# fzaiser/genfer

Measured on AMD Instinct MI355X. Metric: TaylorPoly mul f64 GMAC/s, higher is better.
Workload: dtype f64

## Files before the change

### genfer_amd/csrc/gft_api.hip

```cpp
#include <hip/hip_runtime.h>
#include <dlfcn.h>
#include <rccl/rccl.h>

#include <algorithm>
#include <chrono>
#include <atomic>
#include <cmath>
#include <cstdio>
#include <cstring>
#include <deque>
#include <exception>
#include <functional>
#include <initializer_list>
#include <map>
#include <memory>
#include <tuple>
#include <stdexcept>
#include <string>
#include <vector>

#include "../../include/gftaylor.h"
#include "gft_kernels.hpp"
#include "gft_small_alloc.hpp"
#include "gft_host.hpp"
// ... 1257 lines not shown
        HIP_OK(hipEventSynchronize(R.events[b]));
        float ms = 0;
        HIP_OK(hipEventElapsedTime(&ms, R.events[a], R.events[b]));
        return ms;
    } catch (const std::exception& e) {
        g_err = e.what();
        return -1.0f;
    }
}
int gft_set_option(const char* name, double value) {
    std::string n = name ? name : "";
    if (n == "horner_loop_max") R.horner_loop_max = value < 0 ? 0 : (size_t)value;
    else if (n == "div_wavefront") R.div_wavefront = value != 0;
    else if (n == "exp_right") R.exp_right = value != 0;
    else if (n == "recur_overlap") R.recur_overlap = value != 0;
    else if (n == "defer") R.defer = value != 0;
    else if (n == "lazy_observe") R.lazy_observe = value != 0;
    else if (n == "batch_dag") R.batch_dag = value != 0;
    else if (n == "lazy_horner") R.lazy_horner = value != 0;
    else if (n == "nz_proofs") R.nz_proofs = value != 0;
    else if (n == "lazy_sum") R.lazy_sum = value != 0;
    else if (n == "async_launch") lq_configure(R.device, value != 0);
    else if (n == "trace_lq_report") lq_report();
    else if (n == "shallow_max_terms") R.shallow_max_terms = value < 0 ? 256 : (size_t)value;
    else if (n == "debug_fail_next_launch") g_fail_next_launch.store(value != 0 ? 1 : 0);
    else if (n == "tiled_min_macs") R.tiled_min_macs = value;
    else if (n == "conv_rb_min_macs") staged_set_rb_min_macs(value);
    else if (n == "conv_rb_pairs") staged_set_rb_pairs(value);
    else if (n == "conv_rb_pairs_cap") staged_set_rb_pairs_cap(value);
    else if (n == "conv_rb_pairs_lanes") staged_set_rb_pairs_lanes(value);
    else if (n == "shallow_pair_min") shallow_set_pair_min(value == -1.0 ? 4096.0 : value);
    else if (n == "tiled_tile") tiled_set_lane_tile((int)value);
    else if (n == "tiled_peel") tiled_set_peel((int)value);
    else if (n == "tiled_peel_lanes") tiled_set_peel_lanes((int)value);
    else if (n == "tiled_slots") tiled_set_slots((int)value);
    else if (n == "tiled_taper") tiled_set_taper((int)value);
    else if (n == "host_max_elems") R.host_max_elems = value < 0 ? Runtime::HOST_MAX_ELEMS_DEFAULT : (size_t)value;
    else if (n == "host_max_macs") R.host_max_macs = value < 0 ? Runtime::HOST_MAX_MACS_DEFAULT : value;
    else if (n == "series_form") R.series_force = (value == 1 || value == 2) ? (int)value : 0;
    else if (n == "dist_min_macs") dist_set_min_macs(value);
    else if (n == "dist_event_slot") dist_set_event_slot(value);
    else return -1;
    return 0;
}
int gft_set_conv_variant(int v) {
    R.conv_variant = v;
    return 0;
}
int gft_set_conv_mode(int mode) {
    if (mode < 0 || mode > 3) return -1;
    R.conv_mode = mode;
    return 0;
}

int gft_conv_raw(const double* x, const size_t* xshape, const double* y, const size_t* yshape, double* res,
                 const size_t* rshape, size_t ndim, size_t slab_lo, size_t slab_hi, int accumulate) {
    return guard_int([&] {
        typedef Ops<EF64> O;
        O::HV xv{const_cast<double*>(x), 0, dims(xshape, ndim)};
        O::HV yv{const_cast<double*>(y), 0, dims(yshape, ndim)};
        O::HV zv{res, 0, dims(rshape, ndim)};
        for (size_t i = 0; i < ndim; ++i)
            if (xshape[i] > rshape[i] || yshape[i] > rshape[i] || xshape[i] == 0 || yshape[i] == 0)
                throw Error("conv_raw: operand shapes must be non-empty and not exceed the result shape");
        if (ndim > 0 && (slab_lo > slab_hi || slab_hi > rshape[0])) throw Error("conv_raw: bad slab range");
        O::conv(xv, yv, zv, slab_lo, slab_hi, accumulate != 0, false, 0, 0, 0);
// ... 581 lines not shown
```

### genfer_amd/csrc/gft_conv_tiled.hip

```cpp
#include <algorithm>
#include <cstdio>
#include <cstdlib>
#include <cstring>
#include <map>
#include <vector>

#include "gft_kernels.hpp"
#include "gft_peel_layout.hpp"

namespace gft {

namespace {

struct TileSeg {
    unsigned u, a, b;
    unsigned step_begin, step_end;
    int dest;
};

struct RedTile {
    unsigned u, a, b;
    unsigned first, count;
    unsigned slot0;
};
// ... 13 lines not shown
    unsigned cut;
    unsigned lim1;
    size_t zsU, zs0, zs1, zoff;
    const double* xp;
    const double* yp;
    double* z;
    double* ws;
    const TileSeg* segs;
    const unsigned* wg_begin;
    const RedTile* red;
    const unsigned* red_slots;
    const unsigned* guard;
    unsigned guard_epoch;
    unsigned* claim;
    unsigned n_ranges, n_queues;
#ifdef GFT_TILED_DIAG
    unsigned long long* stamps;
#endif
    unsigned char blk1[8], blk2[8];
};

typedef const double __attribute__((address_space(4))) * cptr_t;

#ifndef GFT_TILED_DEFAULT_VARIANT
#define GFT_TILED_DEFAULT_VARIANT 7
#endif
#ifndef GFT_TILED_PEEL_DEFAULT
#define GFT_TILED_PEEL_DEFAULT -1
#endif
#ifndef GFT_TILED_PEEL_LANES_DEFAULT
#define GFT_TILED_PEEL_LANES_DEFAULT -1
#endif
constexpr unsigned PEEL_MIN_EXTENT = 112, PEEL_MIN_INNER = 64;

__device__ inline void loadx(double (&dst)[8], cptr_t p) {
#pragma unroll
    for (int i = 0; i < 8; ++i) dst[i] = p[i];
}

__device__ inline void load8(double (&dst)[8], const double* p) {
#pragma unroll
    for (int i = 0; i < 8; ++i) dst[i] = p[i];
}

__device__ inline void load8_b128(double (&dst)[8], const double* p) {
    const double2* q = reinterpret_cast<const double2*>(__builtin_assume_aligned(p, 16));
#pragma unroll
    for (int i = 0; i < 4; ++i) {
        double2 v = q[i];
        dst[2 * i] = v.x;
        dst[2 * i + 1] = v.y;
    }
}

__device__ inline void fma_rows(double (&acc)[8], const double (&xq)[8], const double (&cur)[8],
                                const double (&prev)[8], int s_lo, int s_hi) {
#pragma unroll
    for (int s = 0; s < 8; ++s) {
        if (s < s_lo || s >= s_hi) continue;
        const double xs = xq[s];
#pragma unroll
        for (int r = 0; r < 8; ++r) {
            const double yv = (r - s >= 0) ? cur[(r - s) & 7] : prev[(8 + r - s) & 7];
            acc[r] = __builtin_fma(xs, yv, acc[r]);
        }
    }
// ... 449 lines not shown
                                                   double* __restrict__ w0, double* __restrict__ s1, double* __restrict__ w1,
                                                   unsigned n0, unsigned n1, unsigned nI, unsigned n8) {
    const size_t t0 = (size_t)7 * (n0 / 8) * n1 * n8, ts = (size_t)7 * n0 * n8, t1 = (size_t)7 * (n1 / 8) * n0 * n8;
    for (size_t i = blockIdx.x * (size_t)blockDim.x + threadIdx.x; i < t0 + ts + t1; i += (size_t)gridDim.x * blockDim.x) {
        const double* src;
        double* dst;
        size_t row;
        unsigned col;
        if (i < t0) {
            row = i / n8;
            col = (unsigned)(i - row * n8);
            const unsigned r1 = (unsigned)(row % n1), va = (unsigned)(row / n1), a = va % (n0 / 8), v = va / (n0 / 8);
            src = x + ((size_t)(8 * a + 1 + v) * n1 + r1) * nI;
            dst = w0 + i;
        } else if (i < t0 + ts) {
            const size_t k = i - t0;
            row = k / n8;
            col = (unsigned)(k - row * n8);
            const unsigned j1c = (unsigned)(row % n0), ju = (unsigned)(row / n0);
            src = y + ((size_t)j1c * n1 + ju) * nI;
            dst = s1 + k;
        } else {
            const size_t k = i - t0 - ts;
            row = k / n8;
            col = (unsigned)(k - row * n8);
            const unsigned r = (unsigned)(row % n0), vb = (unsigned)(row / n0), b = vb % (n1 / 8), v = vb / (n1 / 8);
            src = x + ((size_t)r * n1 + 8 * b + 1 + v) * nI;
            dst = w1 + k;
        }
        *dst = col < nI ? src[col] : 0.0;
    }
}

__global__ void __launch_bounds__(256) k_pad_rows(const double* __restrict__ in, double* __restrict__ out, size_t rows,
                                                  unsigned len, unsigned P, unsigned B) {
    const size_t per_p = rows * B, total = per_p * P;
    for (size_t i = blockIdx.x * (size_t)blockDim.x + threadIdx.x; i < total; i += (size_t)gridDim.x * blockDim.x) {
        const unsigned p = (unsigned)(i / per_p);
        const size_t rem = i - (size_t)p * per_p, row = rem / B;
        const unsigned col = p * B + (unsigned)(rem - row * B);
        out[i] = col < len ? in[row * len + col] : 0.0;
    }
}
__global__ void __launch_bounds__(256) k_fold_rows(const double* __restrict__ zt, double* __restrict__ z, size_t rows,
                                                   size_t row_lo, size_t row_hi, unsigned Pz, unsigned B, unsigned zI,
                                                   int accumulate, const unsigned* guard, unsigned epoch) {
    if (guard && *guard == epoch) return;
    const unsigned RI = 2 * B - 1;
    size_t total = (row_hi - row_lo) * zI;
    for (size_t i = blockIdx.x * (size_t)blockDim.x + threadIdx.x; i < total; i += (size_t)gridDim.x * blockDim.x) {
        size_t row = row_lo + i / zI;
        unsigned k = (unsigned)(i % zI), p = k / B, r = k - p * B;
        double v = p < Pz ? zt[((size_t)p * rows + row) * RI + r] : 0.0;
        if (p > 0 && p - 1 < Pz && r + 1 < B) v += zt[((size_t)(p - 1) * rows + row) * RI + B + r];
        double* dst = z + row * zI + k;
        *dst = accumulate ? *dst + v : v;
    }
}


struct Variant {
    bool fast;
    bool b128;
    bool xcd;
    bool compact;
    bool peel;
// ... 62 lines not shown
}

unsigned long long& plan_generation() {
    static unsigned long long g = 0;
    return g;
}

void reset_plan_cache(hipStream_t st) {
    (void)hipStreamSynchronize(st);
    for (auto& kv : plan_cache())
        if (kv.second.d_tables) (void)hipFree(kv.second.d_tables);
    plan_cache().clear();
    plan_generation()++;
    arena().head = 0;
}

int num_cus() {
    static int n = 0;
    if (!n) {
        int dev = 0;
        (void)hipGetDevice(&dev);
        hipDeviceProp_t p;
        if (hipGetDeviceProperties(&p, dev) == hipSuccess) n = p.multiProcessorCount;
        if (n <= 0) n = 256;
    }
    return n;
}

struct PeelSpec {
    unsigned role = 0;
    unsigned cut = 0, lim1 = 0;
    size_t zsU = 0, zs0 = 0, zs1 = 0, zoff = 0;
    unsigned all_slabs = 0;
};

int& tiled_slots_cap() {
    static int v = 0;
    return v;
}
#ifndef GFT_TILED_TAPER_DEFAULT
#define GFT_TILED_TAPER_DEFAULT 80
#endif
int& tiled_taper_pct() {
    static int v = GFT_TILED_TAPER_DEFAULT;
    return v;
}

int& tiled_force_tsh() {
    static int v = 0;
    return v;
}

unsigned pick_lane_tile(const TiledArgs& T) {
    auto axis_eff = [](unsigned T, unsigned nx, unsigned ny, unsigned nz) {
        double useful = 0, issued = 0;
        for (unsigned t = 0; t * T < nz; ++t) {
            const unsigned kmax = std::min(T * t + T - 1, nz - 1);
            const unsigned jlo = T * t + 1 > ny ? T * t + 1 - ny : 0, jhi = std::min(kmax + 1, nx);
            if (jhi > jlo) issued += (double)(jhi - jlo) * T;
            for (unsigned k = T * t; k <= kmax; ++k) {
                const unsigned lo = k + 1 > ny ? k + 1 - ny : 0, hi = std::min(k + 1, nx);
                if (hi > lo) useful += hi - lo;
            }
        }
        return issued > 0 ? useful / issued : 0.0;
    };
// ... 275 lines not shown
        case 1: launch_main_nw<1, VAR>(st, P, T, grid); break;
        case 2: launch_main_nw<2, VAR>(st, P, T, grid); break;
        case 4: launch_main_nw<4, VAR>(st, P, T, grid); break;
        default: launch_main_nw<8, VAR>(st, P, T, grid); break;
    }
}

}

void tiled_pad_rows_f64(hipStream_t st, const double* in, double* out, size_t rows, unsigned len, unsigned P, unsigned B) {
    size_t tot = rows * P * B;
    if (!tot) return;
    GFT_LAUNCH(k_pad_rows, dim3((unsigned)std::min<size_t>((tot + 255) / 256, 4096)), dim3(256), 0, st, in, out, rows,
                       len, P, B);
}
void tiled_fold_rows_f64(hipStream_t st, const double* zt, double* z, size_t rows, size_t row_lo, size_t row_hi, unsigned Pz,
                         unsigned B, unsigned zI, int accumulate, const unsigned* guard, unsigned epoch) {
    size_t tot = (row_hi - row_lo) * zI;
    if (!tot) return;
    GFT_LAUNCH(k_fold_rows, dim3((unsigned)std::min<size_t>((tot + 255) / 256, 4096)), dim3(256), 0, st, zt, z, rows,
                       row_lo, row_hi, Pz, B, zI, accumulate, guard, epoch);
}

void tiled_set_lane_tile(int tsh) { tiled_force_tsh() = tsh; }
void tiled_set_slots(int n) { tiled_slots_cap() = n; }
void tiled_set_taper(int pct) { tiled_taper_pct() = pct < 0 ? GFT_TILED_TAPER_DEFAULT : std::min(pct, 90); }

namespace {

int& tiled_peel_mode() {
    static int v = GFT_TILED_PEEL_DEFAULT;
    return v;
}
int& tiled_peel_lanes_mode() {
    static int v = GFT_TILED_PEEL_LANES_DEFAULT;
    return v;
}

const Plan* cached_plan(const ConvArgs& a, const Variant& V, const PeelSpec& ps, hipStream_t st) {
    PlanKey key;
    std::memset(&key, 0, sizeof(key));
    if (a.nd < 2 || a.nd > 4) return nullptr;
    key.v[0] = (unsigned)a.nd | ((unsigned)a.slab_axis << 8) | ((unsigned)tiled_force_tsh() << 16) | ((unsigned)tiled_taper_pct() << 24);
    for (int i = 0; i < a.nd; ++i) {
        key.v[1 + i] = a.xs[i];
        key.v[5 + i] = a.ys[i];
        key.v[9 + i] = a.zs[i];
    }
    key.v[13] = a.slab_lo;
    key.v[14] = a.slab_hi;
    key.v[15] = (unsigned)a.accumulate;
    key.v[16] = (unsigned)(a.j0_min | (a.j0_excl << 8) | (a.j0_desc << 16));
    key.v[17] = V.b128;
    key.v[18] = ps.role | (ps.cut << 4) | (ps.lim1 << 8) | (ps.all_slabs << 12);
    auto& cache = plan_cache();
    auto it = cache.find(key);
    if (it == cache.end()) {
        Plan P;
        if (cache.size() >= 1024) reset_plan_cache(st);
        if (!build_plan(a, V, ps, P, st)) return nullptr;
        it = cache.emplace(key, P).first;
    }
    return &it->second;
}

unsigned launch_grid(const Plan& P) {
    if (tiled_slots_cap() < 0) return P.n_wg;
    unsigned g = std::min(P.n_wg, P.n_resident);
    if (tiled_slots_cap() > 0) g = std::min(g, (unsigned)tiled_slots_cap());
    return g;
}
bool plan_claims(const Plan& P) { return launch_grid(P) < P.n_wg; }
constexpr size_t CLAIM_BYTES = 256;
unsigned* claim_words(char* wb, unsigned launch) { return (unsigned*)wb + 8 * launch; }
void zero_claim_words(hipStream_t st, char* wb) {
    enqueue_task([=] { lq_note((hipMemsetAsync)(wb, 0, CLAIM_BYTES, st), nullptr, "hipMemsetAsync"); });
}

#ifdef GFT_TILED_DIAG
constexpr unsigned STAMP_RANGES = 65536;
unsigned long long* stamp_area(unsigned launch, const Plan& first) {
    static unsigned long long* d_stamps = nullptr;
    const char* stamps_min = std::getenv("GFT_TILED_STAMPS_MIN");
    if (!std::getenv("GFT_TILED_STAMPS") || first.n_wg < (stamps_min ? (unsigned)std::atoi(stamps_min) : 1024u)) return nullptr;
    if (!d_stamps && hipMalloc((void**)&d_stamps, 3 * (size_t)3 * STAMP_RANGES * sizeof(unsigned long long)) != hipSuccess) d_stamps = nullptr;
    return d_stamps ? d_stamps + (size_t)launch * 3 * STAMP_RANGES : nullptr;
}
struct StampedLaunch {
    const char* name;
    const unsigned long long* d_stamps;
    unsigned n, grid;
    bool claiming;
};
void dump_stamps(hipStream_t st, const StampedLaunch* ls, unsigned n_launches) {
    if (hipStreamSynchronize(st) != hipSuccess) return;
    FILE* f = std::fopen(std::getenv("GFT_TILED_STAMPS"), "a");
    if (!f) return;
    unsigned long long first_end = 0;
    for (unsigned l = 0; l < n_launches; ++l) {
        const unsigned n = ls[l].n;
        std::vector<unsigned long long> h(3 * (size_t)n);
        if (!ls[l].d_stamps || hipMemcpy(h.data(), ls[l].d_stamps, h.size() * 8, hipMemcpyDeviceToHost) != hipSuccess) continue;
        unsigned long long t0 = ~0ull, t1 = 0, last[8] = {0}, busy[8] = {0};
        unsigned cnt[8] = {0};
        for (unsigned r = 0; r < n; ++r) {
            const unsigned long long b = h[3 * (size_t)r], e = h[3 * (size_t)r + 1];
            const unsigned x = (unsigned)h[3 * (size_t)r + 2] & 7u;
            t0 = std::min(t0, b);
            t1 = std::max(t1, e);
// ... 80 lines not shown
    o.inplace = operands_slack && B.nx8 == B.xI && B.ny8 == B.yI && B.nxc >= B.nb && B.nyc >= B.nb && !((uintptr_t)y & 15) &&
                !((uintptr_t)x & 7);
    o.pack_y = !o.inplace && (B.ny8 != B.yI || ((uintptr_t)y & 15));
    o.o_ws = claims ? CLAIM_BYTES : 0;
    o.o_xp = o.o_ws + al(n_slots * B.nb * 512 * sizeof(double));
    o.o_yp = o.o_xp + al((x_rows * B.nx8 + 8) * sizeof(double));
    o.end = o.o_yp + al(y_rows * B.ny8 * sizeof(double));
    return o;
}
void bind_operands(hipStream_t st, const Operands& o, const double* x, const double* y, char* wb, unsigned* nf_flag,
                   unsigned nf_epoch, TiledArgs& T) {
    T.ws = (double*)(wb + o.o_ws);
    if (o.inplace) {
        T.xp = x;
        T.yp = y;
        T.guard = nullptr;
        T.guard_epoch = 0;
        return;
    }
    const size_t x_rows = (size_t)T.xU * T.x0 * T.x1, y_rows = (size_t)T.yU * T.y0 * T.y1;
    double *xp = (double*)(wb + o.o_xp), *yp = (double*)(wb + o.o_yp);
    const size_t tot = x_rows * T.nx8 + (o.pack_y ? y_rows * T.ny8 : y_rows * T.yI);
    GFT_LAUNCH(k_prep_operands, dim3((unsigned)std::min<size_t>((tot + 255) / 256, 2048)), dim3(256), 0, st, x, xp, x_rows, T.xI,
               T.nx8, y, o.pack_y ? yp : nullptr, y_rows, T.yI, T.ny8, nf_flag, nf_epoch);
    T.xp = xp;
    T.yp = o.pack_y ? yp : y;
    T.guard = nf_flag;
    T.guard_epoch = nf_epoch;
}

bool peel_applies(const ConvArgs& a, const Variant& V) {
    const int mode = tiled_peel_mode();
    if (mode == 0) return false;
    if (a.nd != 3 || a.slab_axis != 0 || a.slab_lo != 0 || a.slab_hi != a.zs[0]) return false;
    if (a.j0_min || a.j0_excl || a.j0_desc) return false;
    for (int i = 0; i < 3; ++i)
        if (a.xs[i] != a.zs[i] || a.ys[i] != a.zs[i]) return false;
    const unsigned n0 = a.zs[0], n1 = a.zs[1];
    if (n0 % 8 || n1 % 8 || n0 < 16 || n1 < 16 || a.zs[2] > 128) return false;
    if (!V.fast || !V.b128 || V.compact || V.peel || V.other) return false;
    TiledArgs T;
    std::memset(&T, 0, sizeof(T));
    T.x0 = T.y0 = T.z0 = n0;
    T.x1 = T.y1 = T.z1 = n1;
    if (pick_lane_tile(T) != 3) return false;
    return mode == 1 || (n0 >= PEEL_MIN_EXTENT && n1 >= PEEL_MIN_EXTENT && a.zs[2] >= PEEL_MIN_INNER);
}

int conv_tiled_peel(hipStream_t st, const double* x, const double* y, double* z, const ConvArgs& a, const Variant& V, void* ws,
                    size_t ws_bytes, size_t* ws_needed, unsigned* nf_flag, unsigned nf_epoch, bool* guarded, bool* forked) {
    const unsigned n0 = a.zs[0], n1 = a.zs[1], nI = a.zs[2];
    ConvArgs l0, l1;
    std::memset(&l0, 0, sizeof(l0));
    l0.nd = 4;
    l0.slab_lo = 0;
    l0.slab_hi = 7;
    l0.accumulate = 1;
    l1 = l0;
    Variant VL = V;
    VL.peel = true;
    const unsigned s0x[4] = {7, 1, n1, nI}, s0y[4] = {7, n0 / 8, n1, nI}, s1x[4] = {7, 1, n0, nI}, s1y[4] = {7, n1 / 8, n0, nI};
    for (int i = 0; i < 4; ++i) {
        l0.xs[i] = s0x[i]; l0.ys[i] = l0.zs[i] = s0y[i];
        l1.xs[i] = s1x[i]; l1.ys[i] = l1.zs[i] = s1y[i];
    }
    const int lanes_mode = tiled_peel_lanes_mode();
    bool can_fork = lanes_mode != 0 && stream_lanes().ok;
    if (can_fork) {
        hipStreamCaptureStatus cs = hipStreamCaptureStatusNone;
        if (hipStreamIsCapturing(st, &cs) != hipSuccess) (void)hipGetLastError();
        if (cs != hipStreamCaptureStatusNone) can_fork = false;
    }
    bool fork = can_fork && lanes_mode > 0;
    PeelSpec pm, p0, p1;
    pm.role = 1; pm.cut = 3;
    p0.role = 2; p0.zsU = (size_t)n1 * nI; p0.zs0 = 8 * p0.zsU; p0.zs1 = nI; p0.zoff = p0.zsU;
    p1.role = 3; p1.lim1 = 1; p1.zsU = nI; p1.zs0 = 8 * (size_t)nI; p1.zs1 = (size_t)n1 * nI; p1.zoff = nI;
    Plan PM, P0, P1;
    for (int attempt = 0;; ++attempt) {
// ... 54 lines not shown
    T1.yp = w1;
#ifdef GFT_TILED_DIAG
    T.stamps = stamp_area(0, PM);
    T0.stamps = stamp_area(1, PM);
    T1.stamps = stamp_area(2, PM);
#endif
    unsigned *const c = claim_words(wb + L.o_claim, 0), *const c0 = claim_words(wb + L.o_claim, 1), *const c1 = claim_words(wb + L.o_claim, 2);
    if (fork) {
        const bool ok = launch_plan_main(st, PM, T, V, c) && launch_plan_main(st0, P0, T0, VL, c0) && launch_plan_main(st1, P1, T1, VL, c1);
        if (ok) launch_plan_reduce(st, PM, T);
        lanes_join(st);
        if (!ok) return 0;
        launch_plan_reduce(st, P0, T0);
        launch_plan_reduce(st, P1, T1);
    } else {
        if (!launch_plan_main(st, PM, T, V, c)) return 0;
        launch_plan_reduce(st, PM, T);
        if (!launch_plan_main(st, P0, T0, VL, c0)) return 0;
        launch_plan_reduce(st, P0, T0);
        if (!launch_plan_main(st, P1, T1, VL, c1)) return 0;
        launch_plan_reduce(st, P1, T1);
    }
#ifdef GFT_TILED_DIAG
    if (T.stamps) {
        const StampedLaunch ls[3] = {{"M", T.stamps, PM.n_wg, launch_grid(PM), plan_claims(PM)},
                                     {"L0", T0.stamps, P0.n_wg, launch_grid(P0), plan_claims(P0)},
                                     {"L1", T1.stamps, P1.n_wg, launch_grid(P1), plan_claims(P1)}};
        dump_stamps(st, ls, 3);
    }
#endif
    return 1;
}

}

void tiled_set_peel(int mode) { tiled_peel_mode() = mode < 0 ? -1 : (mode ? 1 : 0); }
void tiled_set_peel_lanes(int mode) { tiled_peel_lanes_mode() = mode < 0 ? GFT_TILED_PEEL_LANES_DEFAULT : (mode ? 1 : 0); }

bool conv_tiled_f64(hipStream_t st, const double* x, const double* y, double* z, const ConvArgs& a, void* ws, size_t ws_bytes,
                    size_t* ws_needed, unsigned* nf_flag, unsigned nf_epoch, bool* guarded, bool* peeled, bool* forked) {
    bool compact_operands = false;
    if (a.nd >= 2 && a.nd <= 4) {
        const unsigned nb = (a.zs[a.nd - 1] + 7) / 8;
        compact_operands = (a.xs[a.nd - 1] + 7) / 8 < nb || (a.ys[a.nd - 1] + 7) / 8 < nb;
    }
    const Variant V = decode_variant(a.variant, compact_operands);
    if (peeled) *peeled = false;
    if (forked) *forked = false;
    if (peel_applies(a, V)) {
        const int r = conv_tiled_peel(st, x, y, z, a, V, ws, ws_bytes, ws_needed, nf_flag, nf_epoch, guarded, forked);
        if (r >= 0) {
            if (peeled) *peeled = r == 1;
            return r == 1;
        }
    }
    const Plan* P = cached_plan(a, V, PeelSpec(), st);
    if (!P) return false;
    const bool claims = plan_claims(*P);
    const Operands o = operand_layout(P->base, P->n_slots, claims, x, y, a.operands_slack);
    const size_t need = o.end + 256;
    if (guarded) *guarded = !o.inplace;
    if (ws_needed) *ws_needed = need;
    if (!ws) return true;
    if (ws_bytes < need) return false;
    TiledArgs T = P->base;
    if (claims) zero_claim_words(st, (char*)ws);
    bind_operands(st, o, x, y, (char*)ws, nf_flag, nf_epoch, T);
    T.z = z;
    return launch_plan(st, *P, T, V, claim_words((char*)ws, 0));
}

}
```

### genfer_amd/csrc/gft_kernels.hpp

```cpp
#pragma once
#include <hip/hip_runtime.h>

#include <cstddef>
#include <cstdint>
#include <vector>

#include "gft_elem.hpp"
#include "gft_launch.hpp"
#include "gft_wavefront_plan.hpp"

namespace gft {

constexpr int MAXD = 12;

struct Shape {
    int nd;
    unsigned d[MAXD];
};

struct DView {
    double* p;
    size_t plane;
    Shape sh;
};
// ... 169 lines not shown
    int subtract;
    unsigned total;
};

struct Mailbox {
    double* payload;
    unsigned long long* seq;
    unsigned long long value;
    unsigned* dev_word;
};
__device__ inline void mailbox_publish(const Mailbox& mb) {
    __threadfence_system();
    __hip_atomic_store(mb.seq, mb.value, __ATOMIC_RELEASE, __HIP_MEMORY_SCOPE_SYSTEM);
}
void peek_to_mailbox(hipStream_t st, const double* src, size_t stride, unsigned n, const Mailbox& mb);
void witness_verdict(hipStream_t st, const unsigned* flags, unsigned n, const Mailbox& mb);
void upload_small(hipStream_t st, double* dst, const double* host_src, size_t n);

struct ConvArgs {
    int nd;
    unsigned xs[MAXD], ys[MAXD], zs[MAXD];
    size_t xstr[MAXD], ystr[MAXD], zstr[MAXD];
    unsigned slab_lo, slab_hi;
    int slab_axis;
    int accumulate;
    int j0_min;
    int j0_excl;
    int j0_desc;
    int inner_from_zero;
    int variant;
    int operands_slack;
    const unsigned* guard;
    unsigned guard_epoch;
};

struct ConvEpi {
    int mode;
    unsigned os[MAXD];
    unsigned abox[MAXD];
    size_t astr[MAXD];
    const double* ap;
    size_t aplane;
    unsigned* wit;
};

template <class E>
struct K {
    static void gather(hipStream_t st, const double* src, size_t src_plane, double* out, size_t out_plane,
                       const GatherArgs& a);
    static void chain_copy(hipStream_t st, double* out, size_t out_plane, const Shape& out_shape, const ChainSrc& a);
    static void chain_copy_scan(hipStream_t st, double* out, size_t out_plane, const Shape& out_shape, const ChainSrc& a, unsigned axes_mask,
                                unsigned* state, const Mailbox& mb);
    static void chain_nest(hipStream_t st, double* out, size_t out_plane, const Shape& out_shape, const NestSrc& a, const NestSrc& b, int subtract);
    static void chain_addsub(hipStream_t st, double* out, size_t out_plane, const Shape& out_shape, const ChainSrc& a,
                             const ChainSrc& b, int subtract);
    static void addsub_padded(hipStream_t st, const DView& out, const DView& a, const DView& b, int subtract);
    static void add_scaled_padded(hipStream_t st, const DView& out, const DView& a, const DView& b, Scalar2 c);
    static void copy_first(hipStream_t st, const double* src, size_t src_plane, double* dst, size_t dst_plane, size_t n,
                           int op, const double* s, size_t s_plane, Scalar2 s_value);
    static void set_small(hipStream_t st, double* p, size_t plane, unsigned n, Scalar2 v0, Scalar2 v1);
    static void linear_scan(hipStream_t st, const DView& t, unsigned axes_mask, unsigned* state, const Mailbox& mb);
    static void horner_linear(hipStream_t st, const double* res, size_t res_plane, const double* a, size_t a_plane, double* out,
                              size_t out_plane, const HornerArgs& args);
    static constexpr unsigned HORNER_LINE_MAX = 2048;
    static void horner_linear_loop(hipStream_t st, const double* res0, size_t res0_plane, const double* a, size_t a_plane,
                                   double* out, size_t plane, const HornerLoopArgs& args, unsigned lines, unsigned* wit);
// ... 44 lines not shown
                         unsigned inner, size_t axis_stride_outer, double* out, size_t out_plane, int mode);
    static void any_zero(hipStream_t st, const double* p, size_t plane, size_t n, unsigned* state, const Mailbox& mb);
    static void zero_pattern(hipStream_t st, const double* p, size_t plane, const Shape& sh, size_t n, unsigned* state, const Mailbox& mb);
    static void count_neq(hipStream_t st, const double* a, size_t a_plane, const double* b, size_t b_plane,
                          size_t n, unsigned* count);
    static void conv_naive(hipStream_t st, const double* x, size_t x_plane, const double* y, size_t y_plane,
                           double* z, size_t z_plane, const ConvArgs& a);
    static bool conv_shallow(hipStream_t st, const double* x, size_t x_plane, const double* y, size_t y_plane, double* out,
                             size_t out_plane, const ConvArgs& a, const ConvEpi& e);
    static bool conv_line(hipStream_t st, const double* x, size_t x_plane, const double* y, size_t y_plane, double* z, size_t z_plane,
                          const ConvArgs& a);
};

enum SumMode { SUM_SEQ = 0, SUM_UNROLL8 = 1, SUM_WAVE = 2 };

bool conv_tiled_f64(hipStream_t st, const double* x, const double* y, double* z, const ConvArgs& a, void* ws,
                    size_t ws_bytes, size_t* ws_needed, unsigned* nf_flag, unsigned nf_epoch, bool* guarded = nullptr,
                    bool* peeled = nullptr, bool* forked = nullptr);

template <class E>
bool conv_pairs(hipStream_t st, const double* x, size_t xp, const double* y, size_t yp, double* z, size_t zp, const ConvArgs& a, double max_macs);
void staged_set_rb_min_macs(double v);
void staged_set_rb_pairs(double v);
void staged_set_rb_pairs_cap(double bytes);
void shallow_set_pair_min(double v);
void staged_set_rb_pairs_lanes(double v);
size_t staged_scratch_bytes();
void staged_release_scratch();
void dwf_release_orders();
void tiled_set_lane_tile(int tsh);
void tiled_set_slots(int n);
void tiled_set_taper(int pct);
void tiled_set_peel(int mode);
void tiled_set_peel_lanes(int mode);
void tiled_pad_rows_f64(hipStream_t st, const double* in, double* out, size_t rows, unsigned len, unsigned P, unsigned B);
void tiled_fold_rows_f64(hipStream_t st, const double* zt, double* z, size_t rows, size_t row_lo, size_t row_hi, unsigned Pz,
                         unsigned B, unsigned zI, int accumulate, const unsigned* guard, unsigned epoch);

template <class E>
bool conv_staged(hipStream_t st, const double* x, size_t x_plane, const double* y, size_t y_plane, double* z,
                 size_t z_plane, const ConvArgs& a);

}
```

### genfer_amd/csrc/gft_ops_product.inc

```

    static void conv(const HV& x, const HV& y, const HV& z, size_t slab_lo, size_t slab_hi, bool accumulate,
                     bool slab_mode, int j0_min, int j0_excl, int j0_desc) {
        Dims keep = collapse_mask({&z.shape}, slab_mode);
        Dims xs = pick(x.shape, keep), ys = pick(y.shape, keep), zs = pick(z.shape, keep);
        if (zs.size() > (size_t)MAXD) throw Error("tensor rank exceeds GFT MAXD after collapsing");
        ConvArgs a;
        std::memset(&a, 0, sizeof(a));
        a.nd = (int)zs.size();
        Dims xst = c_strides(xs), yst = c_strides(ys), zst = c_strides(zs);
        for (int i = 0; i < a.nd; ++i) {
            a.xs[i] = (unsigned)xs[i];
            a.ys[i] = (unsigned)ys[i];
            a.zs[i] = (unsigned)zs[i];
            a.xstr[i] = xst[i];
            a.ystr[i] = yst[i];
            a.zstr[i] = zst[i];
        }
        if (!z.shape.empty() && slab_hi <= slab_lo) return;
        const bool axis0_kept = !keep.empty() && keep[0] == 0;
        if (a.nd == 0) {
            a.slab_lo = 0;
            a.slab_hi = 1;
        } else if (!axis0_kept) {
            a.slab_lo = 0;
// ... 139 lines not shown
                return;
            }
            if (R.conv_mode == 2) throw Error("conv_mode=2 (tiled) requested but the shape is not supported by the tiled kernel");
        }
        if (R.conv_mode == 0 || R.conv_mode == 3) {
            if (conv_staged<E>(R.stream, x.p, x.plane, y.p, y.plane, z.p, z.plane, a)) {
                R.stats[4]++;
                return;
            }
        }
        R.stats[5]++;
        K<E>::conv_naive(R.stream, x.p, x.plane, y.p, y.plane, z.p, z.plane, a);
    }

    static bool conv_tiled_high_rank(const HV& x, const HV& y, const HV& z, const ConvArgs& a, const ConvArgs& ash, const double* tx,
                                     const double* ty, double* tz) {
        const int extra = ash.nd - 4;
        ConvArgs sub;
        std::memset(&sub, 0, sizeof(sub));
        sub.nd = 4;
        double macs = 1.0, lead_pairs = 1.0;
        for (int i = 0; i < ash.nd; ++i) macs *= 0.5 * (double)ash.zs[i] * (double)std::min(ash.xs[i], ash.ys[i]);
        for (int i = 0; i < 4; ++i) {
            sub.xs[i] = ash.xs[extra + i];
            sub.ys[i] = ash.ys[extra + i];
            sub.zs[i] = ash.zs[extra + i];
            sub.xstr[i] = ash.xstr[extra + i];
            sub.ystr[i] = ash.ystr[extra + i];
            sub.zstr[i] = ash.zstr[extra + i];
        }
        sub.slab_lo = 0;
        sub.slab_hi = sub.zs[0];
        sub.variant = ash.variant;
        for (int i = 0; i < extra; ++i) lead_pairs *= 0.5 * (double)ash.zs[i] * (double)std::min(ash.xs[i], ash.ys[i]) + 0.5;
        if (R.conv_mode == 0 && macs / lead_pairs < R.tiled_min_macs) return false;
        size_t need = 0;
        if (!conv_tiled_f64(R.stream, tx, ty, tz, sub, nullptr, 0, &need, nullptr, 0)) return false;
        R.ensure_conv_ws(need);
        unsigned* flag = R.next_nf_epoch();
        unsigned u[MAXD] = {0}, j[MAXD] = {0};
        for (int i = 0; i < extra; ++i) u[i] = i == 0 ? ash.slab_lo : 0;
        const unsigned u0_hi = ash.slab_hi;
        if (u0_hi <= ash.slab_lo) return true;
        for (;;) {
            size_t zoff = 0;
            unsigned jlo[MAXD], jhi[MAXD];
            bool any = true;
            for (int i = 0; i < extra; ++i) {
                zoff += (size_t)u[i] * ash.zstr[i];
                jlo[i] = u[i] + 1 > ash.ys[i] ? u[i] + 1 - ash.ys[i] : 0;
                jhi[i] = std::min(u[i], ash.xs[i] - 1);
                if (jlo[i] > jhi[i]) any = false;
                j[i] = jlo[i];
            }
            bool first = true;
            if (!any) {
                zero_elems(false, tz + zoff, (size_t)ash.zstr[extra - 1]);
            } else {
                for (;;) {
                    size_t xoff = 0, yoff = 0;
                    for (int i = 0; i < extra; ++i) {
                        xoff += (size_t)j[i] * ash.xstr[i];
                        yoff += (size_t)(u[i] - j[i]) * ash.ystr[i];
                    }
                    sub.accumulate = first ? 0 : 1;
                    first = false;
// ... 113 lines not shown
```

### genfer_amd/csrc/gft_peel_layout.hpp

```cpp
#pragma once
#include <cstddef>

namespace gft {

constexpr size_t PEEL_ALIGN = 256;
constexpr size_t PEEL_CLAIM_BYTES = 256;
constexpr size_t PEEL_SLAB_DOUBLES = 512;

struct PeelLayout {
    size_t o_claim, o_slab[3], o_xp, o_yp, o_w0, o_s1, o_w1;
    size_t b_claim, b_slab[3], b_xp, b_yp, b_w0, b_s1, b_w1;
    size_t need;
};

inline size_t peel_align(size_t v) { return (v + PEEL_ALIGN - 1) / PEEL_ALIGN * PEEL_ALIGN; }

inline PeelLayout peel_layout(const size_t (&slots)[3], size_t nb, bool claims, size_t xp_doubles, size_t yp_doubles, size_t w0_doubles,
                              size_t s1_doubles, size_t w1_doubles) {
    PeelLayout L;
    size_t at = 0;
    auto put = [&at](size_t bytes, size_t& off, size_t& len) {
        off = at;
        len = bytes;
        at += peel_align(bytes);
    };
    put(claims ? PEEL_CLAIM_BYTES : 0, L.o_claim, L.b_claim);
    for (int i = 0; i < 3; ++i) put(slots[i] * nb * PEEL_SLAB_DOUBLES * sizeof(double), L.o_slab[i], L.b_slab[i]);
    put(xp_doubles * sizeof(double), L.o_xp, L.b_xp);
    put(yp_doubles * sizeof(double), L.o_yp, L.b_yp);
    put(w0_doubles * sizeof(double), L.o_w0, L.b_w0);
    put(s1_doubles * sizeof(double), L.o_s1, L.b_s1);
    put(w1_doubles * sizeof(double), L.o_w1, L.b_w1);
    L.need = at + PEEL_ALIGN;
    return L;
}

inline PeelLayout peel_layout_for(const size_t (&slots)[3], size_t n0, size_t n1, size_t n8, bool claims) {
    const size_t rows = n0 * n1;
    return peel_layout(slots, n8 / 8, claims, rows * n8 + 8, rows * n8, 7 * (n0 / 8) * n1 * n8, 7 * n0 * n8 + 8, 7 * (n1 / 8) * n0 * n8);
}

}
```

Measured before the change: 31090.

## Add peeled tiled convolution path for 4-D f64 series products

Extends the peeled tiled convolution scheme from 3-D to 4-D operands. A main aligned-block launch is followed by per-stripe L-shaped remainder launches along two axes, each fed by a packing kernel that gathers the boundary rows into padded buffers. Inner calls from the leading-axis loop set no_peel so they keep the old path. The aim is to run the bulk of the 4-D product in the fast 8-aligned tiled kernel instead of per-slab sub-convolutions. In exchange it adds many extra launches, pack traffic and a larger workspace.

Result: no change. 31070 (-0.0%).

```diff
diff --git a/genfer_amd/csrc/gft_api.hip b/genfer_amd/csrc/gft_api.hip
--- a/genfer_amd/csrc/gft_api.hip
+++ b/genfer_amd/csrc/gft_api.hip
@@ -1313,6 +1313,7 @@
     else if (n == "shallow_pair_min") shallow_set_pair_min(value == -1.0 ? 4096.0 : value);
     else if (n == "tiled_tile") tiled_set_lane_tile((int)value);
     else if (n == "tiled_peel") tiled_set_peel((int)value);
+    else if (n == "tiled_peel4") tiled_set_peel4((int)value);
     else if (n == "tiled_peel_lanes") tiled_set_peel_lanes((int)value);
     else if (n == "tiled_slots") tiled_set_slots((int)value);
     else if (n == "tiled_taper") tiled_set_taper((int)value);
diff --git a/genfer_amd/csrc/gft_conv_tiled.hip b/genfer_amd/csrc/gft_conv_tiled.hip
--- a/genfer_amd/csrc/gft_conv_tiled.hip
+++ b/genfer_amd/csrc/gft_conv_tiled.hip
@@ -69,6 +69,7 @@
 #define GFT_TILED_PEEL_LANES_DEFAULT -1
 #endif
 constexpr unsigned PEEL_MIN_EXTENT = 112, PEEL_MIN_INNER = 64;
+constexpr unsigned PEEL4_MIN_LEAD = 48, PEEL4_MIN_EXTENT = 32, PEEL4_MIN_INNER = 16;
 
 __device__ inline void loadx(double (&dst)[8], cptr_t p) {
 #pragma unroll
@@ -584,6 +585,34 @@
     }
 }
 
+__global__ void __launch_bounds__(256) k_pack_peel4(const double* __restrict__ x, const double* __restrict__ y,
+                                                    double* __restrict__ s0, double* __restrict__ s1, double* __restrict__ w,
+                                                    Peel4Shape sh, unsigned nI, unsigned n8, unsigned part, unsigned t) {
+    const size_t r0 = (size_t)7 * sh.nU * sh.n1, r1 = (size_t)7 * sh.nU * sh.n0;
+    const size_t e0 = (part == 2 ? r1 : r0) * n8, e1 = part ? e0 : e0 + r1 * n8;
+    for (size_t i = blockIdx.x * (size_t)blockDim.x + threadIdx.x; i < e1; i += (size_t)gridDim.x * blockDim.x) {
+        const double* src;
+        double* dst;
+        size_t k = i;
+        if (part == 1) {
+            src = x + peel4_w0_src(sh, t * r0 + k / n8) * nI;
+            dst = w;
+        } else if (part == 2) {
+            src = x + peel4_w1_src(sh, t * r1 + k / n8) * nI;
+            dst = w;
+        } else if (i < e0) {
+            src = y + peel4_s0_src(sh, k / n8) * nI;
+            dst = s0;
+        } else {
+            k = i - e0;
+            src = y + peel4_s1_src(sh, k / n8) * nI;
+            dst = s1;
+        }
+        const unsigned col = (unsigned)(k % n8);
+        dst[k] = col < nI ? src[col] : 0.0;
+    }
+}
+
 __global__ void __launch_bounds__(256) k_pad_rows(const double* __restrict__ in, double* __restrict__ out, size_t rows,
                                                   unsigned len, unsigned P, unsigned B) {
     const size_t per_p = rows * B, total = per_p * P;
@@ -712,6 +741,7 @@
     unsigned cut = 0, lim1 = 0;
     size_t zsU = 0, zs0 = 0, zs1 = 0, zoff = 0;
     unsigned all_slabs = 0;
+    unsigned ext = 0;
 };
 
 int& tiled_slots_cap() {
@@ -1053,6 +1083,10 @@
     static int v = GFT_TILED_PEEL_DEFAULT;
     return v;
 }
+int& tiled_peel4_mode() {
+    static int v = -1;
+    return v;
+}
 int& tiled_peel_lanes_mode() {
     static int v = GFT_TILED_PEEL_LANES_DEFAULT;
     return v;
@@ -1073,7 +1107,7 @@
     key.v[15] = (unsigned)a.accumulate;
     key.v[16] = (unsigned)(a.j0_min | (a.j0_excl << 8) | (a.j0_desc << 16));
     key.v[17] = V.b128;
-    key.v[18] = ps.role | (ps.cut << 4) | (ps.lim1 << 8) | (ps.all_slabs << 12);
+    key.v[18] = ps.role | (ps.cut << 4) | (ps.lim1 << 8) | (ps.all_slabs << 12) | (ps.ext << 16);
     auto& cache = plan_cache();
     auto it = cache.find(key);
     if (it == cache.end()) {
@@ -1094,8 +1128,8 @@
 bool plan_claims(const Plan& P) { return launch_grid(P) < P.n_wg; }
 constexpr size_t CLAIM_BYTES = 256;
 unsigned* claim_words(char* wb, unsigned launch) { return (unsigned*)wb + 8 * launch; }
-void zero_claim_words(hipStream_t st, char* wb) {
-    enqueue_task([=] { lq_note((hipMemsetAsync)(wb, 0, CLAIM_BYTES, st), nullptr, "hipMemsetAsync"); });
+void zero_claim_words(hipStream_t st, char* wb, size_t bytes = CLAIM_BYTES) {
+    enqueue_task([=] { lq_note((hipMemsetAsync)(wb, 0, bytes, st), nullptr, "hipMemsetAsync"); });
 }
 
 #ifdef GFT_TILED_DIAG
@@ -1242,19 +1276,22 @@
 bool peel_applies(const ConvArgs& a, const Variant& V) {
     const int mode = tiled_peel_mode();
     if (mode == 0) return false;
-    if (a.nd != 3 || a.slab_axis != 0 || a.slab_lo != 0 || a.slab_hi != a.zs[0]) return false;
+    if ((a.nd != 3 && a.nd != 4) || a.no_peel || a.slab_axis != 0 || a.slab_lo != 0 || a.slab_hi != a.zs[0]) return false;
     if (a.j0_min || a.j0_excl || a.j0_desc) return false;
-    for (int i = 0; i < 3; ++i)
+    for (int i = 0; i < a.nd; ++i)
         if (a.xs[i] != a.zs[i] || a.ys[i] != a.zs[i]) return false;
-    const unsigned n0 = a.zs[0], n1 = a.zs[1];
-    if (n0 % 8 || n1 % 8 || n0 < 16 || n1 < 16 || a.zs[2] > 128) return false;
+    const unsigned n0 = a.zs[a.nd - 3], n1 = a.zs[a.nd - 2], nI = a.zs[a.nd - 1];
+    if (n0 % 8 || n1 % 8 || n0 < 16 || n1 < 16 || nI > 128) return false;
     if (!V.fast || !V.b128 || V.compact || V.peel || V.other) return false;
     TiledArgs T;
     std::memset(&T, 0, sizeof(T));
     T.x0 = T.y0 = T.z0 = n0;
     T.x1 = T.y1 = T.z1 = n1;
     if (pick_lane_tile(T) != 3) return false;
-    return mode == 1 || (n0 >= PEEL_MIN_EXTENT && n1 >= PEEL_MIN_EXTENT && a.zs[2] >= PEEL_MIN_INNER);
+    if (a.nd == 4 && tiled_peel4_mode() >= 0) return tiled_peel4_mode() == 1;
+    if (a.nd == 3 && mode == 1) return true;
+    if (a.nd == 4) return n0 >= PEEL4_MIN_EXTENT && n1 >= PEEL4_MIN_EXTENT && nI >= PEEL4_MIN_INNER && a.zs[0] >= PEEL4_MIN_LEAD;
+    return n0 >= PEEL_MIN_EXTENT && n1 >= PEEL_MIN_EXTENT && nI >= PEEL_MIN_INNER;
 }
 
 int conv_tiled_peel(hipStream_t st, const double* x, const double* y, double* z, const ConvArgs& a, const Variant& V, void* ws,
@@ -1375,9 +1412,92 @@
     return 1;
 }
 
+int conv_tiled_peel4(hipStream_t st, const double* x, const double* y, double* z, const ConvArgs& a, const Variant& V, void* ws,
+                     size_t ws_bytes, size_t* ws_needed, unsigned* nf_flag, unsigned nf_epoch, bool* guarded) {
+    const unsigned nU = a.zs[0], n0 = a.zs[1], n1 = a.zs[2], nI = a.zs[3];
+    if (n0 > 0xffffu || n1 > 0xffffu) return -1;
+    ConvArgs l0, l1;
+    std::memset(&l0, 0, sizeof(l0));
+    l0.nd = 4;
+    l0.slab_lo = 0;
+    l0.slab_hi = 7;
+    l0.accumulate = 1;
+    l1 = l0;
+    Variant VL = V;
+    VL.peel = true;
+    const unsigned s0[4] = {7, nU, n1, nI}, s1[4] = {7, nU, n0, nI};
+    for (int i = 0; i < 4; ++i) {
+        l0.xs[i] = l0.ys[i] = l0.zs[i] = s0[i];
+        l1.xs[i] = l1.ys[i] = l1.zs[i] = s1[i];
+    }
+    PeelSpec pm, p0, p1;
+    pm.role = 1; pm.cut = 3;
+    const Peel4Out o0 = peel4_out(0, 0, n0, n1, nI), o1 = peel4_out(1, 0, n0, n1, nI);
+    p0.role = 4; p0.ext = n0; p0.zsU = o0.zsU; p0.zs0 = o0.zs0; p0.zs1 = o0.zs1; p0.zoff = o0.zoff;
+    p1.role = 5; p1.ext = n1; p1.lim1 = 1; p1.zsU = o1.zsU; p1.zs0 = o1.zs0; p1.zs1 = o1.zs1; p1.zoff = o1.zoff;
+    Plan PM, P0, P1;
+    for (int attempt = 0;; ++attempt) {
+        const unsigned long long gen = plan_generation();
+        const Plan* q = cached_plan(a, V, pm, st);
+        if (!q) return -1;
+        PM = *q;
+        if (!(q = cached_plan(l0, VL, p0, st))) return -1;
+        P0 = *q;
+        if (!(q = cached_plan(l1, VL, p1, st))) return -1;
+        P1 = *q;
+        if (gen == plan_generation()) break;
+        if (attempt) return -1;
+    }
+    const TiledArgs& B = PM.base;
+    if (B.tsh != 3) return -1;
+    Operands o = operand_layout(B, 0, true, x, y, a.operands_slack);
+    const Peel4Layout L = peel4_layout(PM.n_slots, std::max(P0.n_slots, P1.n_slots), nU, n0, n1, B.nx8);
+    o.o_ws = L.o_slab[0];
+    o.o_xp = L.o_xp;
+    o.o_yp = L.o_yp;
+    if (ws && ws_bytes < L.need) return -1;
+    if (ws_needed) *ws_needed = L.need;
+    if (guarded) *guarded = !o.inplace;
+    if (!ws) return 1;
+
+    char* wb = (char*)ws;
+    double *g_s0 = (double*)(wb + L.o_s0), *g_s1 = (double*)(wb + L.o_s1), *g_w = (double*)(wb + L.o_w);
+    TiledArgs T = B;
+    zero_claim_words(st, wb + L.o_claim, L.b_claim);
+    bind_operands(st, o, x, y, wb, nf_flag, nf_epoch, T);
+    const Peel4Shape sh = {nU, n0, n1};
+    auto pack = [&](unsigned part, unsigned t, size_t rows) {
+        GFT_LAUNCH(k_pack_peel4, dim3((unsigned)std::min<size_t>((rows * B.nx8 + 255) / 256, 4096)), dim3(256), 0, st, x, y, g_s0, g_s1, g_w, sh,
+                   nI, B.nx8, part, t);
+    };
+    pack(0, 0, L.rows_s0 + L.rows_s1);
+    T.z = z;
+    unsigned launch = 0;
+    if (!launch_plan_main(st, PM, T, V, claim_words(wb + L.o_claim, launch++))) return 0;
+    launch_plan_reduce(st, PM, T);
+    for (int axis = 0; axis < 2; ++axis) {
+        const Plan& PL = axis ? P1 : P0;
+        for (unsigned t = 0; t < (axis ? n1 : n0) / 8; ++t) {
+            TiledArgs TL = PL.base;
+            TL.ws = (double*)(wb + L.o_slab[1]);
+            TL.z = z;
+            TL.guard = T.guard;
+            TL.guard_epoch = T.guard_epoch;
+            TL.xp = axis ? g_s1 : g_s0;
+            TL.yp = g_w;
+            TL.zoff = peel4_out(axis, t, n0, n1, nI).zoff;
+            pack(1 + axis, t, axis ? L.rows_w1 : L.rows_w0);
+            if (!launch_plan_main(st, PL, TL, VL, claim_words(wb + L.o_claim, launch++))) return 0;
+            launch_plan_reduce(st, PL, TL);
+        }
+    }
+    return 1;
+}
+
 }
 
 void tiled_set_peel(int mode) { tiled_peel_mode() = mode < 0 ? -1 : (mode ? 1 : 0); }
+void tiled_set_peel4(int mode) { tiled_peel4_mode() = mode < 0 ? -1 : (mode ? 1 : 0); }
 void tiled_set_peel_lanes(int mode) { tiled_peel_lanes_mode() = mode < 0 ? GFT_TILED_PEEL_LANES_DEFAULT : (mode ? 1 : 0); }
 
 bool conv_tiled_f64(hipStream_t st, const double* x, const double* y, double* z, const ConvArgs& a, void* ws, size_t ws_bytes,
@@ -1391,7 +1511,8 @@
     if (peeled) *peeled = false;
     if (forked) *forked = false;
     if (peel_applies(a, V)) {
-        const int r = conv_tiled_peel(st, x, y, z, a, V, ws, ws_bytes, ws_needed, nf_flag, nf_epoch, guarded, forked);
+        const int r = a.nd == 4 ? conv_tiled_peel4(st, x, y, z, a, V, ws, ws_bytes, ws_needed, nf_flag, nf_epoch, guarded)
+                                : conv_tiled_peel(st, x, y, z, a, V, ws, ws_bytes, ws_needed, nf_flag, nf_epoch, guarded, forked);
         if (r >= 0) {
             if (peeled) *peeled = r == 1;
             return r == 1;
diff --git a/genfer_amd/csrc/gft_kernels.hpp b/genfer_amd/csrc/gft_kernels.hpp
--- a/genfer_amd/csrc/gft_kernels.hpp
+++ b/genfer_amd/csrc/gft_kernels.hpp
@@ -225,6 +225,7 @@
     int operands_slack;
     const unsigned* guard;
     unsigned guard_epoch;
+    int no_peel;
 };
 
 struct ConvEpi {
@@ -335,6 +336,7 @@
 void tiled_set_slots(int n);
 void tiled_set_taper(int pct);
 void tiled_set_peel(int mode);
+void tiled_set_peel4(int mode);
 void tiled_set_peel_lanes(int mode);
 void tiled_pad_rows_f64(hipStream_t st, const double* in, double* out, size_t rows, unsigned len, unsigned P, unsigned B);
 void tiled_fold_rows_f64(hipStream_t st, const double* zt, double* z, size_t rows, size_t row_lo, size_t row_hi, unsigned Pz,
diff --git a/genfer_amd/csrc/gft_ops_product.inc b/genfer_amd/csrc/gft_ops_product.inc
--- a/genfer_amd/csrc/gft_ops_product.inc
+++ b/genfer_amd/csrc/gft_ops_product.inc
@@ -195,6 +195,7 @@
         sub.slab_lo = 0;
         sub.slab_hi = sub.zs[0];
         sub.variant = ash.variant;
+        sub.no_peel = 1;
         for (int i = 0; i < extra; ++i) lead_pairs *= 0.5 * (double)ash.zs[i] * (double)std::min(ash.xs[i], ash.ys[i]) + 0.5;
         if (R.conv_mode == 0 && macs / lead_pairs < R.tiled_min_macs) return false;
         size_t need = 0;
diff --git a/genfer_amd/csrc/gft_peel_layout.hpp b/genfer_amd/csrc/gft_peel_layout.hpp
--- a/genfer_amd/csrc/gft_peel_layout.hpp
+++ b/genfer_amd/csrc/gft_peel_layout.hpp
@@ -40,4 +40,73 @@
     return peel_layout(slots, n8 / 8, claims, rows * n8 + 8, rows * n8, 7 * (n0 / 8) * n1 * n8, 7 * n0 * n8 + 8, 7 * (n1 / 8) * n0 * n8);
 }
 
+#if defined(__HIPCC__)
+#define GFT_PEEL_HD __host__ __device__
+#else
+#define GFT_PEEL_HD
+#endif
+
+struct Peel4Shape {
+    size_t nU, n0, n1;
+};
+GFT_PEEL_HD inline size_t peel4_s0_src(const Peel4Shape& s, size_t row) {
+    const size_t j1 = row % s.n1, dj = row / s.n1, jU = dj % s.nU, d = dj / s.nU;
+    return (jU * s.n0 + d) * s.n1 + j1;
 }
+GFT_PEEL_HD inline size_t peel4_s1_src(const Peel4Shape& s, size_t row) {
+    const size_t j0 = row % s.n0, dj = row / s.n0, jU = dj % s.nU, d = dj / s.nU;
+    return (jU * s.n0 + j0) * s.n1 + d;
+}
+GFT_PEEL_HD inline size_t peel4_w0_src(const Peel4Shape& s, size_t row) {
+    const size_t r = row % s.n1, t = row / s.n1, U = t % s.nU, ae = t / s.nU, e = ae % 7, a = ae / 7;
+    return (U * s.n0 + 8 * a + 1 + e) * s.n1 + r;
+}
+GFT_PEEL_HD inline size_t peel4_w1_src(const Peel4Shape& s, size_t row) {
+    const size_t r = row % s.n0, t = row / s.n0, U = t % s.nU, be = t / s.nU, e = be % 7, b = be / 7;
+    return (U * s.n0 + r) * s.n1 + 8 * b + 1 + e;
+}
+
+struct Peel4Out {
+    size_t zsU, zs0, zs1, zoff;
+};
+GFT_PEEL_HD inline Peel4Out peel4_out(int axis, size_t t, size_t n0, size_t n1, size_t nI) {
+    const size_t s1 = nI, s0 = n1 * nI, sU = n0 * s0;
+    return axis ? Peel4Out{s1, sU, s0, (8 * t + 1) * s1} : Peel4Out{s0, sU, s1, (8 * t + 1) * s0};
+}
+
+struct Peel4Layout {
+    size_t o_claim, o_slab[2], o_xp, o_yp, o_s0, o_s1, o_w;
+    size_t b_claim, b_slab[2], b_xp, b_yp, b_s0, b_s1, b_w;
+    size_t rows_s0, rows_s1, rows_w0, rows_w1;
+    size_t need;
+};
+constexpr size_t PEEL_CLAIM_WORDS = 8;
+
+inline size_t peel4_launches(size_t n0, size_t n1) { return 1 + n0 / 8 + n1 / 8; }
+
+inline Peel4Layout peel4_layout(size_t slots_m, size_t slots_l, size_t nU, size_t n0, size_t n1, size_t n8) {
+    Peel4Layout L;
+    size_t at = 0;
+    auto put = [&at](size_t bytes, size_t& off, size_t& len) {
+        off = at;
+        len = bytes;
+        at += peel_align(bytes);
+    };
+    const size_t rows = nU * n0 * n1, slab = n8 / 8 * PEEL_SLAB_DOUBLES * sizeof(double);
+    L.rows_s0 = 7 * nU * n1;
+    L.rows_s1 = 7 * nU * n0;
+    L.rows_w0 = 7 * nU * n1;
+    L.rows_w1 = 7 * nU * n0;
+    put(peel4_launches(n0, n1) * PEEL_CLAIM_WORDS * sizeof(unsigned), L.o_claim, L.b_claim);
+    put(slots_m * slab, L.o_slab[0], L.b_slab[0]);
+    put(slots_l * slab, L.o_slab[1], L.b_slab[1]);
+    put((rows * n8 + 8) * sizeof(double), L.o_xp, L.b_xp);
+    put(rows * n8 * sizeof(double), L.o_yp, L.b_yp);
+    put((L.rows_s0 * n8 + 8) * sizeof(double), L.o_s0, L.b_s0);
+    put((L.rows_s1 * n8 + 8) * sizeof(double), L.o_s1, L.b_s1);
+    put((L.rows_w0 > L.rows_w1 ? L.rows_w0 : L.rows_w1) * n8 * sizeof(double), L.o_w, L.b_w);
+    L.need = at + PEEL_ALIGN;
+    return L;
+}
+
+}
```
